# junipertcy/bipartiteSBM-MCMC

Measured on AMD Instinct MI355X. Metric: node-label MH updates/s, higher is better.
Workload: dtype f64

## Files before the change

bipartitesbm-mcmc_amd/build.py:

```python
import os
import shutil
import subprocess
import sys

HERE = os.path.dirname(os.path.abspath(__file__))
CSRC = os.path.join(HERE, "csrc")
LIB = os.path.join(HERE, "libbisbm_hip.so")
SOURCES = ["bisbm_kernels.hip", "bisbm_sweep_fast.hip", "bisbm_handle.hip", "bisbm_anneal.hip", "bisbm_marginals.hip",
           "bisbm_multi.hip", "bisbm_merge.hip", "bisbm_align.hip", "bisbm_tempering.hip", "bisbm_population.hip", "bisbm_pair_scores.hip", "bisbm_partition.hip",
           "bisbm_query_scores.hip", "bisbm_coassign.hip", "bisbm_foldin.hip", "bisbm_conditionals.hip", "bisbm_heatbath.hip", "bisbm_reshuffle.hip",
           "bisbm_mode_marginals.hip", "bisbm_trace.hip",
           "bisbm_tables.cpp", "bisbm_io.cpp"]
HEADERS = ["bisbm_device.hpp", "bisbm_partition_device.hpp", "bisbm_kernels.hpp", "bisbm_stand_rule.hpp", "bisbm_engine.hpp", "bisbm_pass_policy.hpp", os.path.join("..", "host", "bisbm.hpp"),
           os.path.join("..", "host", "mcmc_main.cpp"), os.path.join("..", "..", "include", "bisbm.h"),
           os.path.join("..", "..", "include", "bisbm_io.h")]
FLAGS = ["--offload-arch=gfx950", "-O3", "-std=c++17", "-ffp-contract=off", "-fPIC", "-pthread",
         "-Wall", "-Wno-unused-function",
         "-mllvm", "-structurizecfg-skip-uniform-regions=true",
         "-mllvm", "-amdgpu-atomic-optimizer-strategy=None",
         "-falign-loops=64"]


def hipcc():
    for cand in (shutil.which("hipcc"), "/opt/rocm/bin/hipcc"):
        if cand and os.path.exists(cand):
            return cand
    raise RuntimeError("hipcc not found: the engine is HIP-only and cannot be built without ROCm")


def needs_build():
    if not os.path.exists(LIB):
        return True
    t = os.path.getmtime(LIB)
    deps = [os.path.join(CSRC, s) for s in SOURCES + HEADERS] + [os.path.abspath(__file__)]
    return any(os.path.getmtime(d) > t for d in deps)


def build(force=False, verbose=False):
    import fcntl
    if not force and not needs_build():
        return LIB
    with open(os.path.join(HERE, ".build.lock"), "w") as lock:
        fcntl.flock(lock, fcntl.LOCK_EX)
        try:
            if not force and not needs_build():
                return LIB
# ... 100 lines not shown
```

bipartitesbm-mcmc_amd/csrc/bisbm_anneal.hip:

```cpp
#include "bisbm_engine.hpp"

using namespace bisbm;

extern "C" {

int bisbm_anneal(bisbm_handle h, int schedule, const float kwargs[2], uint64_t duration_steps,
                 uint64_t steps_await, double* acc_rate_out) {
    if (!h) return BISBM_ERR_INVALID_ARG;
    if (h->temper.L)
        return fail(h, BISBM_ERR_STATE, "replica exchange is on: sweeps run through bisbm_tempering_run (bisbm_tempering_set(h, 0, NULL) turns it off)");
    return anneal_engine(h, schedule, kwargs, duration_steps, steps_await, acc_rate_out, nullptr);
}

}

int bisbm::anneal_engine(bisbm_engine* h, int schedule, const float kwargs[2], uint64_t duration_steps, uint64_t steps_await,
                         double* acc_rate_out, const float* T_chain) {
    if (!kwargs) return fail(h, BISBM_ERR_INVALID_ARG, "kwargs is NULL");
    if (schedule < BISBM_SCHED_EXPONENTIAL || schedule > BISBM_SCHED_ABRUPT_COOL)
        return fail(h, BISBM_ERR_INVALID_ARG, "unknown schedule %d", schedule);
    if (!h->devs.empty()) return multi_anneal(h, schedule, kwargs, duration_steps, steps_await, acc_rate_out);
    if (!h->groups.empty()) {
        const size_t G = h->groups.size();
        std::vector<int> rcs(G, BISBM_OK);
// ... 181 lines not shown
            Slice sl;
            sl.T = schedule_table(sched, k0, k1, t0, len, &sl.zero_after);
            return sl;
        });
    };
    if (tab_segments) start_slice(0, slice_sweeps(sweeps_left));
    bool first = true;
    while (first || sweeps_left > 0) {
        if (segmented) {
            const uint64_t now = slice_sweeps(sweeps_left);
            p.duration = now * h->n;
            p.t_base = sweeps_done * h->n;
            p.resume = first ? 0u : 1u;
            if (tab_segments) {
                Slice sl;
                try {
                    sl = next_slice.get();
                } catch (...) {
                    return fail(h, BISBM_ERR_STATE, "temperature table: out of host memory");
                }
                if (int rc = upload_table(sl.T, p.t_base, sl.zero_after)) return rc;
            }
            sweeps_left -= now;
            sweeps_done += now;
        }
        first = false;
        uint32_t depth = max_depth;
        if (max_depth >= 2u) {
            depth = h->passes.choose(max_depth, h->n <= 100000);
            if (const char* pd = getenv("BISBM_PASS_DEPTH"))
                depth = pd[0] == '2' ? 1u : pd[0] == '4' ? std::min(2u, max_depth) : pd[0] == '8' ? max_depth : depth;
        }
        p.pass_depth = depth;
        {
            const uint32_t d = std::min(p.pair_steps, p.pass_depth);
            const bool cold = schedule == SCHED_CONSTANT && kwargs[0] == 0.f;
            h->last_pass_steps = (!fast || cold) ? 1u
                                 : (h->ka <= 8 && h->kb <= 8 && d >= 3u) ? 8u
                                 : (h->ka <= 32 && h->kb <= 32 && d >= 2u) ? 4u
                                 : p.pair_steps != 0u ? 2u : 1u;
        }
        HIPCHK(h, hipEventRecord(h->ev0, h->stream));
        if (fast)
            HIPCHK(h, launch_sweep_fast(p, lds, h->stream));
        else
            HIPCHK(h, launch_sweep(p, h->rng_mode, lds, h->stream));
        HIPCHK(h, hipEventRecord(h->ev1, h->stream));
        if (tab_segments && sweeps_left > 0) start_slice(sweeps_done, slice_sweeps(sweeps_left));
        HIPCHK(h, hipStreamSynchronize(h->stream));
        float ms = 0;
        HIPCHK(h, hipEventElapsedTime(&ms, h->ev0, h->ev1));
        ms_sum += ms;
        HIPCHK(h, hipMemcpy(sc.data(), h->d_scalars, sizeof(ChainScalars) * h->n_chains, hipMemcpyDeviceToHost));
        uint64_t upd = 0;
        bool all_stopped = true;
        for (uint32_t c = 0; c < h->n_chains; ++c) {
            acc_sum[c] += sc[c].last_accepted;
            sweeps_sum[c] += sc[c].last_sweeps;
            upd += sc[c].last_sweeps * h->n;
            all_stopped = all_stopped && sc[c].stopped != 0;
        }
        updates += upd;
        if (max_depth >= 2u && ms > 0.05f && upd > 0) {
            const double speed = (double)upd / ms;
            uint64_t acc_now = 0;
            for (uint32_t c = 0; c < h->n_chains; ++c) acc_now += sc[c].last_accepted;
            const double acc_frac = (double)acc_now / (double)upd;
            const double before[3] = {h->passes.figure(1), h->passes.figure(2), h->passes.figure(3)};
            const uint32_t incumbent = h->passes.current();
            h->passes.record(depth, speed, acc_frac);
            if (getenv("BISBM_PASS_LOG"))
                fprintf(stderr, "[bisbm passes] depth %u%s: %.3e updates/ms, accepted %.3f (before the launch: two %.3e, four %.3e, eight %.3e; incumbent %u -> %u)\n",
                        depth, depth != incumbent && incumbent != 0u && h->passes.settled() ? " (a look)" : "", speed, acc_frac, before[0], before[1], before[2],
                        incumbent, h->passes.current());
        }
        if (segmented && fast && all_stopped) {
            if (next_slice.valid()) next_slice.wait();
            break;
        }
    }
    const float ms = (float)ms_sum;
    h->last_kernel_ms = ms_sum;
    if (segmented) {
        for (uint32_t c = 0; c < h->n_chains; ++c) {
            sc[c].last_accepted = acc_sum[c];
            sc[c].last_sweeps = sweeps_sum[c];
            sc[c].last_rate = (fast && sc[c].stopped) ? (double)acc_sum[c] / (double)(sweeps_sum[c] * h->n)
                                                      : (double)acc_sum[c] / (double)duration_steps;
        }
        HIPCHK(h, hipMemcpy(h->d_scalars, sc.data(), sizeof(ChainScalars) * h->n_chains, hipMemcpyHostToDevice));
    }
    if (sum_from_entropy) {
        if (int rc = launch_block_entropy(h, h->d_tmp_f64)) return rc;
        HIPCHK(h, launch_sum_from_entropy(h->d_scalars, h->d_ent_prev, h->d_tmp_f64, h->n_chains, h->stream));
        HIPCHK(h, hipMemcpyAsync(h->d_ent_prev, h->d_tmp_f64, sizeof(double) * h->n_chains, hipMemcpyDeviceToDevice, h->stream));
        HIPCHK(h, hipStreamSynchronize(h->stream));
        h->ent_prev_valid = true;
    }
    for (uint32_t c = 0; c < h->n_chains; ++c)
        if (acc_rate_out) acc_rate_out[c] = sc[c].last_rate;
// ... 23 lines not shown
```

bipartitesbm-mcmc_amd/csrc/bisbm_engine.hpp:

```cpp
#pragma once

#include <hip/hip_runtime.h>

#include <algorithm>
#include <atomic>
#include <cmath>
#include <cstdarg>
#include <cstdio>
#include <cstdlib>
#include <cstring>
#include <future>
#include <limits>
#include <map>
#include <memory>
#include <mutex>
#include <queue>
#include <random>
#include <set>
#include <sstream>
#include <string>
#include <thread>
#include <utility>
#include <vector>

// ... 287 lines not shown
    uint8_t* d_labels_tmp = nullptr;
    size_t label_stride = 0;
    bool wide = false;
    size_t lbytes() const { return wide ? 2 : 1; }
    uint32_t* d_vlist = nullptr;
    int32_t* d_m = nullptr;
    int32_t* d_m_r = nullptr;
    int32_t* d_n_r = nullptr;
    uint32_t* d_eta = nullptr;
    bisbm::ChainScalars* d_scalars = nullptr;
    uint32_t* d_simd_claims = nullptr;
    uint32_t* d_mt_engine = nullptr;
    uint32_t* d_mt_gen = nullptr;
    double* d_lgamma = nullptr;
    double* d_logtab = nullptr;
    double* d_q = nullptr;
    bisbm::DeviceBuf<double> d_T;
    double* d_tmp_f64 = nullptr;
    double* d_ent_prev = nullptr;
    bool ent_prev_valid = false;
    uint32_t* d_stage_u32 = nullptr;
    uint32_t* d_counts = nullptr;
    uint32_t counts_kmax = 0;
    uint32_t counts_cols = 0;
    uint32_t cap_ka = 0, cap_kb = 0;
    std::shared_ptr<bisbm::HostTables> tab;
    uint32_t q_stride = 0;
    double ent_deg = 0, ent_multi = 0;
    std::shared_ptr<std::vector<uint64_t>> deg_count;
    double last_kernel_ms = 0;
    uint64_t last_updates = 0;
    uint32_t last_pass_steps = 0;
    bisbm::PassDepthPolicy passes;
    std::vector<bisbm_engine*> groups;
    std::vector<std::pair<uint32_t, uint32_t>> where;
    bisbm_engine* root = nullptr;
    std::vector<uint32_t> gids, ridx;
    uint32_t* d_gids = nullptr;
    uint32_t gid(size_t c) const { return gids.empty() ? first_chain_id + (uint32_t)c : gids[c]; }
    std::vector<bisbm_engine*> devs;
    std::vector<uint32_t> dev_first;
    struct DevicePool* pool = nullptr;
    uint64_t counts_rows = 0;
    bisbm::AlignState align;
    bisbm::TemperState temper;
    bisbm::PopulationState population;
    bisbm::PairScoreState pairs;
    bisbm::QueryScoreState queries;
    bisbm::CoassignState coassign;
    bisbm::FoldinState foldin;
    bisbm::ConditionalState cond;
    bisbm::ReshuffleState reshuffle;
    bisbm::PartitionState partition;
    bisbm::ModeState modes;
    bisbm::TraceState trace;
};

namespace bisbm {

extern thread_local std::string g_create_error;

int fail(bisbm_engine* h, int code, const char* fmt, ...) __attribute__((format(printf, 3, 4)));

#define HIPCHK(h, expr)                                                                              \
    do {                                                                                             \
        hipError_t e_ = (expr);                                                                      \
        if (e_ != hipSuccess) return fail((h), BISBM_ERR_HIP, "%s: %s", #expr, hipGetErrorString(e_)); \
    } while (0)

#define RESERVE(h, buf, count)                                                                                                \
    do {                                                                                                                      \
        const size_t n_ = (count);                                                                                            \
        hipError_t e_ = (buf).reserve(n_);                                                                                    \
        if (e_ != hipSuccess)                                                                                                 \
            return fail((h), BISBM_ERR_HIP, "%s: %zu bytes of device memory for " #buf " could not be allocated: %s", __func__, \
                        n_ * sizeof(*(buf).get()), hipGetErrorString(e_));                                                    \
    } while (0)

void free_chain_arrays(bisbm_engine* h);
void free_all(bisbm_engine* h);
void mt_seed_host(uint32_t* mt, uint64_t seed);
inline void philox_host(uint64_t seed, uint32_t chain, uint32_t purpose, uint64_t idx, uint32_t out[4]) {
    uint32_t c0 = (uint32_t)idx, c1 = (uint32_t)(idx >> 32), c2 = chain, c3 = purpose;
    uint32_t k0 = (uint32_t)seed, k1 = (uint32_t)(seed >> 32);
    for (int r = 0; r < 10; ++r) {
        const uint64_t p0 = (uint64_t)0xD2511F53u * c0, p1 = (uint64_t)0xCD9E8D57u * c2;
        const uint32_t n0 = (uint32_t)(p1 >> 32) ^ c1 ^ k0, n2 = (uint32_t)(p0 >> 32) ^ c3 ^ k1;
        c1 = (uint32_t)p1;
        c3 = (uint32_t)p0;
        c0 = n0;
        c2 = n2;
        k0 += 0x9E3779B9u;
        k1 += 0xBB67AE85u;
    }
    out[0] = c0, out[1] = c1, out[2] = c2, out[3] = c3;
}
inline double u53_host(uint32_t hi, uint32_t lo) { return (double)((((uint64_t)hi << 32) | lo) >> 11) * 0x1.0p-53; }
inline void forget_pass_speeds(bisbm_engine* h) { h->passes.reset(); }
int rebuild_state(bisbm_engine* h);
int launch_block_entropy(bisbm_engine* h, double* d_out);

template <class F>
int each_group(bisbm_engine* h, F f) {
    for (bisbm_engine* g : h->groups) {
        const int rc = f(g);
        if (rc) {
            h->err = g->err;
            return rc;
        }
    }
    return BISBM_OK;
}
bool common_shape(bisbm_engine* h);
int shared_shape(bisbm_engine* h, uint32_t* ka, uint32_t* kb);
template <class T, class F>
int gather_groups(bisbm_engine* h, T* out, F f) {
    return each_group(h, [&](bisbm_engine* g) {
        std::vector<T> tmp(g->n_chains);
        const int rc = f(g, tmp.data());
        if (rc == BISBM_OK && out)
            for (size_t j = 0; j < tmp.size(); ++j) out[g->ridx[j]] = tmp[j];
        return rc;
    });
}

size_t generic_lds_base_bytes(uint32_t ka, uint32_t kb, bool wide, int rng_mode);
constexpr size_t kLdsPerCu = 160 * 1024;

template <class F>
bool for_each_chain(size_t C, F&& fn) {
    std::atomic<bool> ok{true};
// ... 130 lines not shown
```

bipartitesbm-mcmc_amd/csrc/bisbm_kernels.hpp:

```cpp
#pragma once

#include <hip/hip_runtime.h>
#include <stdint.h>

#include "bisbm_device.hpp"

struct bisbm_reshuffle_record;

namespace bisbm {

struct ChainScalars {
    double cum_dS;
    double accu_r;
    double last_rate;
    uint64_t sweeps_total;
    uint64_t last_accepted;
    uint64_t last_sweeps;
    uint32_t shuffle_epoch;
    uint32_t engine_idx;
    uint32_t gen_idx;
    uint32_t merge_epoch;
    uint32_t hw_id[2];
    uint32_t xcc_id;
    uint32_t split_epoch;
// ... 13 lines not shown
    const uint32_t* chain_gids;
    uint8_t* labels;
    size_t label_stride;
    uint32_t* vlist;
    int32_t* m;
    int32_t* m_r;
    int32_t* n_r;
    uint32_t* eta;
    ChainScalars* scalars;
    uint32_t* mt_engine;
    uint32_t* mt_gen;
    const double* lgamma_tab;
    uint64_t lgamma_size;
    const double* q_tab;
    uint32_t q_stride;
    const double* log_tab;
    const double* T_tab;
    uint64_t T_len;
    uint64_t T_base;
    int T_zero_after;
    int schedule;
    float kw0, kw1;
    uint64_t duration, steps_await;
    uint64_t t_base, call_duration;
    uint32_t resume;
    uint64_t seed;
    int eta_in_lds;
    uint32_t eta_w, eta_lo_a, eta_lo_b;
    int vlist_in_lds;
    uint32_t* simd_claims;
    uint32_t fixed_stepping_wave;
    uint32_t pair_steps;
    uint32_t pass_depth;
    uint32_t wide;
    uint32_t keep_sum;
    const float* T_chain;
};
constexpr uint32_t kSimdClaims = 1u << 14;

struct BuildParams {
    const uint32_t* rowptr;
    const uint32_t* col;
    uint32_t n, na, ka, kb, maxdeg, n_chains;
    const uint8_t* labels;
    size_t label_stride;
    int32_t* m;
    int32_t* m_r;
    int32_t* n_r;
    uint32_t* eta;
    uint32_t wide;
};

struct ShuffleParams {
    uint32_t n, na, nb, n_chains, first_chain_id;
    const uint32_t* chain_gids;
    uint64_t seed;
    uint8_t* labels;
    const uint8_t* labels_old;
    size_t label_stride;
    ChainScalars* scalars;
    uint32_t* mt_engine;
    uint32_t wide;
};

struct EntropyParams {
    uint32_t ka, kb, maxdeg, n_chains;
    const int32_t* m;
    const int32_t* m_r;
    const int32_t* n_r;
    const uint32_t* eta;
// ... 373 lines not shown
```

bipartitesbm-mcmc_amd/csrc/bisbm_sweep_fast.hip:

```cpp
#include "bisbm_kernels.hpp"
#include "bisbm_stand_rule.hpp"

#include <algorithm>
#include <cstdio>
#include <type_traits>

namespace bisbm {

#ifdef BISBM_STAMPS
__device__ unsigned long long g_fast_stamps[16];
#define FSTAMP(i)                                                                        \
    do {                                                                                 \
        unsigned long long now_;                                                         \
        __builtin_amdgcn_sched_barrier(0);                                               \
        __asm__ volatile("s_memtime %0\n\ts_waitcnt lgkmcnt(0)" : "=s"(now_)::"memory"); \
        __builtin_amdgcn_sched_barrier(0);                                               \
        st_acc[i] += now_ - st_prev;                                                     \
        st_prev = now_;                                                                  \
    } while (0)
#else
#define FSTAMP(i) \
    do {          \
    } while (0)
#endif
#if defined(BISBM_STAMPS) && BISBM_STAMPS == 2
#define FSTAMP_STEP(i) \
    do {               \
    } while (0)
#else
#define FSTAMP_STEP(i) FSTAMP(i)
#endif

__device__ __forceinline__ void wfence() {
    __builtin_amdgcn_wave_barrier();
    __asm__ volatile("" ::: "memory");
}

__device__ __forceinline__ double tab_at(const double* base, uint32_t idx) {
#if defined(BISBM_ABLATE) && (BISBM_ABLATE & 8)
    return (double)idx * 1e-3 + (double)((size_t)base & 0xff);
#endif
    return *(const double*)((const char*)base + (uint32_t)(idx << 3));
}

struct __attribute__((packed, aligned(4))) Id4 {
    uint32_t x, y, z, w;
};

__device__ __forceinline__ uint32_t sflag(uint32_t x) {
    uint32_t r;
    __asm__("s_min_u32 %0, %1, 1" : "=s"(r) : "s"(x) : "scc");
    return r;
}
__device__ __forceinline__ uint32_t smin(uint32_t x, uint32_t y) {
    uint32_t r;
    __asm__("s_min_u32 %0, %1, %2" : "=s"(r) : "s"(x), "s"(y) : "scc");
    return r;
}


#ifdef BISBM_PASS_COUNTS
constexpr int kPassCounts = 13;
__device__ unsigned long long g_pass_counts[kPassCounts];
#define PCOUNT(i, v) (pc_acc[i] += (v))
#define PASS_COUNTS_PAIR(paired)                                                          \
    do {                                                                                  \
        const uint32_t pm_ = (paired) & chA, colk_ = col & sflag(kAtB) & (set_clash ^ 1u); \
        const uint32_t mv_ = target_moves(margin, kAtB);                                  \
        pc_acc[0] += 1u;                                                                  \
        pc_acc[1] += 1u + stands;                                                         \
        pc_acc[2] += pm_;                                                                 \
        pc_acc[3] += pm_ & set_clash;                                                     \
        pc_acc[4] += pm_ & colk_ & (mv_ ^ 1u);                                            \
        pc_acc[5] += pm_ & colk_ & mv_;                                                   \
        pc_acc[6] += pm_ & colk_ & (margin == kAtB ? 1u : 0u);                            \
        pc_acc[7] += pm_ & colk_ & (margin + 1u == kAtB ? 1u : 0u);                       \
    } while (0)
#else
#define PCOUNT(i, v) \
    do {             \
    } while (0)
#define PASS_COUNTS_PAIR(paired) \
    do {                         \
    } while (0)
#endif

#ifndef BISBM_PREDICT_TARGET
#define BISBM_PREDICT_TARGET 1
#endif
constexpr uint32_t kHistStride = 68;
constexpr uint32_t kHandWords = 9;
// ... 16 lines not shown
    double logn, tail_lg, L2_0, L2_1, L4_0, L4_1;
};

struct PairSteps {
    uint32_t r_locA, r_locB, degA, degB, t_locB, s_prdA, s_prdB;
    uint32_t liveA, liveB;
    uint32_t selfA, selfB, warmA, warmB;
    uint32_t prop, pack_v, deg, r_loc, t_loc;
    double u_acc;
    __device__ __forceinline__ uint32_t flags(uint32_t clash) const {
        return (liveA & (selfA ^ 1u)) | ((liveA & selfA & warmA) << 1) | ((liveB & (selfB ^ 1u)) << 2) | ((liveB & selfB & warmB) << 3) |
               (clash << 4);
    }
};

__device__ __forceinline__ uint32_t rows4(unsigned long long b) {
    const unsigned long long x = b >> 15;
    return (uint32_t)(x | (x >> 15) | (x >> 30) | (x >> 45)) & 0xfu;
}
__device__ __forceinline__ void commit_four(uint32_t nst, uint32_t clash_bits, uint32_t mv4, uint32_t& moved, uint32_t& commit) {
    const uint32_t c01 = (clash_bits >> 1) & 1u, c02 = (clash_bits >> 2) & 1u, c03 = (clash_bits >> 3) & 1u;
    const uint32_t c12 = (clash_bits >> 6) & 1u, c13 = (clash_bits >> 7) & 1u, c23 = (clash_bits >> 11) & 1u;
    const uint32_t m0 = mv4 & 1u;
    const uint32_t k1 = sflag(nst - 1u) & ((m0 & c01) ^ 1u);
    const uint32_t m1 = k1 & (mv4 >> 1) & 1u;
    const uint32_t k2 = k1 & (nst > 2u ? 1u : 0u) & ((m0 & c02) ^ 1u) & ((m1 & c12) ^ 1u);
    const uint32_t m2 = k2 & (mv4 >> 2) & 1u;
    const uint32_t k3 = k2 & (nst > 3u ? 1u : 0u) & ((m0 & c03) ^ 1u) & ((m1 & c13) ^ 1u) & ((m2 & c23) ^ 1u);
    const uint32_t m3 = k3 & (mv4 >> 3) & 1u;
    commit = 1u | (k1 << 1) | (k2 << 2) | (k3 << 3);
    moved = m0 | (m1 << 1) | (m2 << 2) | (m3 << 3);
}

template <bool EL, bool CT, bool K32, bool K16, bool K8, bool Q32>
__global__ __launch_bounds__(2 * kWave, 2) void sweep_fast_kernel(SweepParams p) {
    extern __shared__ __align__(16) uint32_t lds32[];
    const uint32_t chain = blockIdx.x;
    if (chain >= p.n_chains) return;
    const uint32_t lane = threadIdx.x & 63u;
    if (p.resume != 0u && p.scalars[chain].stopped != 0u) {
        if (threadIdx.x == 0) {
            p.scalars[chain].last_accepted = 0;
            p.scalars[chain].last_sweeps = 0;
        }
        return;
    }
    const uint32_t ka = p.ka, kb = p.kb, K = ka + kb, na = p.na, nb = p.nb;
    const uint32_t D = p.maxdeg + 1, S = kb | 1u;
    constexpr bool kPredictTarget = !K16 && !Q32 && (BISBM_PREDICT_TARGET != 0);
    const uint32_t row_cap = p.maxdeg < kRowCap ? p.maxdeg : kRowCap;
    const uint32_t o_mq = 0, o_eta = ka * S;
    const uint32_t eta_w = EL ? D : p.eta_w;
    const uint32_t o_hist8 = o_eta + (EL ? K * D : (ka > kb ? ka : kb) * eta_w);
    const uint32_t o_hand = o_hist8 + 2 * kWave * (kHistStride / 4);
    const uint32_t o_slow = o_hand + 2 * kHandWords * kWave;
    const uint32_t o_flag = o_slow + kWave;
    int32_t* const mq = (int32_t*)(lds32 + o_mq);
    uint32_t* const eta_l = lds32 + o_eta;
    uint32_t* const hist8_base = lds32 + o_hist8;
    uint32_t* const hand_base = lds32 + o_hand;
    int32_t* const slow_hist = (int32_t*)(lds32 + o_slow);
    uint32_t* const stop_flag = lds32 + o_flag;
    unsigned long long* const below1_total = (unsigned long long*)(lds32 + ((o_flag + 4u + 1u) & ~1u));
    const uint32_t wave_in_wg = (uint32_t)__builtin_amdgcn_readfirstlane((int)(threadIdx.x >> 6));
    uint32_t hw_id, xcc_id;
    __asm__ volatile("s_getreg_b32 %0, hwreg(HW_REG_HW_ID)" : "=s"(hw_id));
    __asm__ volatile("s_getreg_b32 %0, hwreg(HW_REG_XCC_ID)" : "=s"(xcc_id));
    uint32_t* const role = lds32 + o_flag + 1;
// ... 726 lines not shown
                    const uint32_t r_i = (uint32_t)__builtin_amdgcn_ds_bpermute(li, (int)r_c);
                    const uint32_t s_i = (uint32_t)__builtin_amdgcn_ds_bpermute(li, (int)s_c);
                    const uint32_t r_j = (uint32_t)__builtin_amdgcn_ds_bpermute(lj, (int)r_c);
                    const uint32_t s_j = (uint32_t)__builtin_amdgcn_ds_bpermute(lj, (int)s_c);
                    const uint32_t t_j = (uint32_t)__builtin_amdgcn_ds_bpermute(lj, (int)t_c);
                    const int at_sj = lj + (int)((s_j & 15u) << 2);
                    const uint32_t margins_j = (uint32_t)__builtin_amdgcn_ds_bpermute(at_sj, (int)m_c);
                    const uint32_t k_i_tj = k_of_i_at(li, t_j);
                    const uint32_t set_i = (1u << r_i) | (1u << s_i), set_j = (1u << r_j) | (1u << s_j);
                    const uint32_t in_between = column_clash<DEPTH>(r_i, s_i, s_j, k_i_tj, margins_j);
#ifdef BISBM_PASS_COUNTS
                    {
                        const uint32_t shared = (set_i & set_j) != 0u ? 1u : 0u;
                        const uint32_t cand = column_clash_any(r_i, s_i, s_j, k_i_tj) & (shared ^ 1u);
                        const uint32_t margin = packed_margin(margins_j, r_i < s_i ? 1u : 0u), need = (DEPTH - 1u) * k_i_tj;
                        pc_pair_code = shared | (cand << 1) | ((cand & in_between) << 2) | ((cand & (need == margin ? 1u : 0u)) << 3) |
                                       ((cand & (need == margin + 1u ? 1u : 0u)) << 4);
                    }
#endif
                    return __builtin_amdgcn_ballot_w64(((set_i & set_j) | in_between) != 0u);
                };
#ifdef BISBM_PASS_COUNTS
                auto count_pairs = [&](uint32_t i, uint32_t j, bool pair_lane, uint32_t moved, uint32_t commit, uint32_t nst) {
                    const bool on = pair_lane && i < j && j < nst && ((moved >> i) & 1u) != 0u && ((commit >> ((j - 1u) & 7u)) & 1u) != 0u;
                    const uint32_t c = on ? pc_pair_code : 0u;
                    pc_acc[8] += (unsigned)__builtin_popcountll(__builtin_amdgcn_ballot_w64((c & 1u) != 0u));
                    pc_acc[9] += (unsigned)__builtin_popcountll(__builtin_amdgcn_ballot_w64((c & 6u) == 2u));
                    pc_acc[10] += (unsigned)__builtin_popcountll(__builtin_amdgcn_ballot_w64((c & 6u) == 6u));
                    pc_acc[11] += (unsigned)__builtin_popcountll(__builtin_amdgcn_ballot_w64((c & 8u) != 0u));
                    pc_acc[12] += (unsigned)__builtin_popcountll(__builtin_amdgcn_ballot_w64((c & 16u) != 0u));
                };
#endif
                auto apply_moves = [&](auto tm, auto width, uint32_t q, uint32_t qs, uint32_t grp_l, uint32_t moved, uint32_t selfok, uint32_t r_loc,
                                       uint32_t s_loc, uint32_t deg, double dS, uint32_t e_idx, int ee, auto&& write_mq) {
                    constexpr bool TM = decltype(tm)::value;
                    constexpr uint32_t W = decltype(width)::value, L = 64u / W;
                    constexpr unsigned long long kFirst = W == 4u ? 0x0001000100010001ull : 0x0101010101010101ull;
                    acc_chunk += (uint32_t)__builtin_popcount(moved | selfok);
                    if ((TM ? (moved | selfok) : moved) != 0u) {
                        const unsigned long long movers = __builtin_amdgcn_ballot_w64(((moved >> grp_l) & 1u) != 0u);
                        wfence();
                        write_mq(movers);
                        if (__builtin_amdgcn_inverse_ballot_w64(movers & (kFirst * 0x30ull)))
                            eta_l[e_idx] = (uint32_t)(ee + ((int)(lb & 1u) * 2 - 1));
                        if (__builtin_amdgcn_inverse_ballot_w64(movers & kFirst)) new_lab[qs] = (uint8_t)(own_base + s_loc);
#pragma unroll
                        for (uint32_t g = 0; g < W; ++g) {
                            if ((moved >> g) & 1u) {
                                const uint32_t rg = readlane(r_loc, L * g), sg = readlane(s_loc, L * g), dg = readlane(deg, L * g);
                                const int dl = (int)min(lb ^ rg, 1u) - (int)min(lb ^ sg, 1u);
                                mr_own += __mul24((int)dg, dl);
                                nr_own += dl;
                                if constexpr (TM) cum_l0 += readlane(dS, L * g + L - 1u);
                                if constexpr (TM) new_minimum(q + g);
                            } else if (TM && ((selfok >> g) & 1u)) {
                                new_minimum(q + g);
                            }
                        }
                        wfence();
                    }
                };
                auto multi_loop = [&](auto tm, auto width, auto&& pass) {
                    constexpr uint32_t W = decltype(width)::value;
                    uint32_t q = 0;
                    acc_chunk = 0;
                    while (q < cnt) {
                        const uint32_t some = (uint32_t)(gen_mask >> q) & ((1u << W) - 1u);
                        if (__builtin_expect((some & 1u) != 0u, 0)) {
                            step_general(q, T_of_step(q));
                            q += 1u;
                        } else {
                            const uint32_t nst = min(min((uint32_t)__builtin_ctz(some | (1u << W)), W), cnt - q);
                            const uint32_t done = pass(tm, q, nst);
                            PCOUNT(0, 1u);
                            PCOUNT(1, done);
                            q += done;
                        }
                    }
                    acc_l0 += (unsigned long long)acc_chunk;
                };

                auto step_pair = [&](auto tm, uint32_t q, uint32_t pairable) -> uint32_t {
                    const uint32_t qB = q + pairable;
                    const uint32_t qs = q + ((uint32_t)half_mask_l & pairable);
                    FSTAMP_STEP(0);
                    PairSteps P = pair_head(q, qB, qs, pairable);
                    const uint32_t r_locA = P.r_locA, s_prdA = P.s_prdA, r_locB = P.r_locB, s_prdB = P.s_prdB, t_locB = P.t_locB;
                    const uint32_t prop = P.prop, deg = P.deg, r_loc = P.r_loc, t_loc = P.t_loc;
                    const int k = (int)hist8_cur[qs * kHistStride + lb];
// ... 222 lines not shown
                    const unsigned long long m_warm = CT ? ~0ull : ~__builtin_amdgcn_ballot_w64(((zeroT_mask >> qs) & 1ull) != 0ull);
                    const unsigned long long b_can = m_valid & m_live & ~m_self & kRowRep;
                    const unsigned long long b_selfok = m_valid & m_live & m_self & m_warm & kRowRep;
                    if (b_can == 0ull) {
                        acc_chunk += (uint32_t)__builtin_popcountll(b_selfok);
                        if constexpr (TM)
                            if (b_selfok != 0ull) new_minimum(q + ((uint32_t)__builtin_ctzll(b_selfok) >> 4));
                        return nst;
                    }
                    TargetReads t;
                    target_lds(t, s_loc, r_loc, deg, kmask);
                    target_gathers(t, kk, std::false_type{});
                    const double a0 = k * (t.m_st + eps) * inv_blk;
                    const double a1 = k * (m_rt - k + eps) * inv_blk;
                    const double accu0 = butterfly_rows16(a0);
                    const double accu1 = butterfly_rows16(a1);
                    const double lq = hot_log_q(std::true_type{}, t.qn, t.qk, t.logn);
                    const uint32_t clash_bits =
                        (uint32_t)clash_pairs(Four{}, r_loc, s_loc, t_loc, pack_margins(margin_up((uint32_t)scan, (uint32_t)w_piv, prop), margin_down((uint32_t)scan, prop)),
                                              (int)(((lane >> 2) & 3u) << 6), (int)((lane & 3u) << 6), [&](int li, uint32_t t_j) {
                            return (uint32_t)__builtin_amdgcn_ds_bpermute(li + (int)(t_j << 2), (int)kk);
                        }) & 0xffffu;
                    double d = (L1 + t.L2) - (L3 + t.L4);
                    d = d + t.tail_lg * sign_tail;
                    d = d + lq * sign_q;
                    const double dS = butterfly_rows16(d);
                    const unsigned long long b_acc = accept_rows(dS, accu0, accu1, u_acc, qs, m_warm, b_can);
                    const uint32_t mv4 = rows4(b_can & b_acc), selfok4 = rows4(b_selfok);
                    uint32_t moved, commit;
                    commit_four(nst, clash_bits, mv4, moved, commit);
#ifdef BISBM_PASS_COUNTS
                    count_pairs((lane >> 2) & 3u, lane & 3u, lane < 16u, moved, commit, nst);
#endif
                    apply_moves(tm, Four{}, q, qs, row, moved, commit & selfok4, r_loc, s_loc, deg, dS, t.e_idx, t.ee, [&](unsigned long long movers) {
                        if (__builtin_amdgcn_inverse_ballot_w64(movers & lanes_koth)) {
                            mq[a_rt] = m_rt_raw - k;
                            mq[t.a_st] = t.m_st_raw + k;
                        }
                    });
                    return (uint32_t)__builtin_popcount(commit);
                };
                auto step_quad32 = [&](auto tm, uint32_t q, uint32_t nst) -> uint32_t {
                    constexpr bool TM = decltype(tm)::value;
                    const uint32_t qs = q + min(row, nst - 1u);
                    const int sel = (int)(qs << 2);
                    const uint32_t prop = prop_of(qs);
                    const uint32_t pack = (uint32_t)__builtin_amdgcn_ds_bpermute(sel, (int)pack_l);
                    const double u_acc = u_acc_of(qs);
                    const uint32_t deg = pack & 255u, r_loc = (pack >> 8) & 63u, t_loc = (pack >> 16) & 63u;
                    const int k0 = (int)hist8_cur[qs * kHistStride + l16], k1 = (int)hist8_cur[qs * kHistStride + l16 + 16u];
                    const uint32_t a_rt0 = mq_at(r_loc, l16), a_rt1 = mq_at(r_loc, l16 + 16u);
                    const int32_t m_rt_raw0 = mq[a_rt0], m_rt_raw1 = mq[a_rt1];
                    const int w0 = mq[mq_at(l16, t_loc)], w1 = mq[mq_at(l16 + 16u, t_loc)];
                    const int nn_r = __builtin_amdgcn_ds_bpermute((int)(r_loc << 2), nr_own);
                    const int32_t kmask0 = (0 - k0) >> 31, kmask1 = (0 - k1) >> 31;
                    const int32_t m_rt0 = m_rt_raw0 & kmask0, m_rt1 = m_rt_raw1 & kmask1;
                    const uint32_t kk0 = (uint32_t)k0, kk1 = (uint32_t)k1;
                    const double L1_0 = tab_at(tab.lg, (uint32_t)(m_rt0 + 1)), L3_0 = tab_at(tab.lg, (uint32_t)(m_rt0 + 1) - kk0);
                    const double L1_1 = tab_at(tab.lg, (uint32_t)(m_rt1 + 1)), L3_1 = tab_at(tab.lg, (uint32_t)(m_rt1 + 1) - kk1);
                    __asm__ volatile("" ::: "memory");
                    const int scan0 = row_inclusive_scan16(w0);
                    int tot = w0;
                    tot += __builtin_amdgcn_update_dpp(0, tot, kDppXor1, 0xF, 0xF, false);
                    tot += __builtin_amdgcn_update_dpp(0, tot, kDppXor2, 0xF, 0xF, false);
                    tot += __builtin_amdgcn_update_dpp(0, tot, kDppHalfMirror, 0xF, 0xF, false);
                    tot += __builtin_amdgcn_update_dpp(0, tot, kDppMirror, 0xF, 0xF, false);
                    const int scan1 = row_inclusive_scan16(w1) + tot;
// ... 4 lines not shown
                    const unsigned long long m_valid = nst >= 4u ? ~0ull : ((1ull << (16u * nst)) - 1ull);
                    const unsigned long long m_live = __builtin_amdgcn_ballot_w64(nn_r != 1);
                    const unsigned long long m_self = __builtin_amdgcn_ballot_w64(s_loc == r_loc);
                    const unsigned long long m_warm = CT ? ~0ull : ~__builtin_amdgcn_ballot_w64(((zeroT_mask >> qs) & 1ull) != 0ull);
                    const unsigned long long b_can = m_valid & m_live & ~m_self & kRowRep;
                    const unsigned long long b_selfok = m_valid & m_live & m_self & m_warm & kRowRep;
                    if (b_can == 0ull) {
                        acc_chunk += (uint32_t)__builtin_popcountll(b_selfok);
                        if constexpr (TM)
                            if (b_selfok != 0ull) new_minimum(q + ((uint32_t)__builtin_ctzll(b_selfok) >> 4));
                        return nst;
                    }
                    TargetReads2 t;
                    target_lds2(t, s_loc, r_loc, deg, kmask0, kmask1, l16, 16u);
                    target_gathers2(t, kk0, kk1, std::true_type{});
                    const uint32_t leaf_m = 0u - (s_loc >> 4);
                    const uint32_t S_own = (uint32_t)scan0 ^ (((uint32_t)scan0 ^ (uint32_t)scan1) & leaf_m);
                    const uint32_t w_own = (uint32_t)w0 ^ (((uint32_t)w0 ^ (uint32_t)w1) & leaf_m);
                    uint32_t margins = pack_margins(margin_up(S_own, w_own, prop), margin_down(S_own, prop));
                    __asm__ volatile("" : "+v"(margins));
                    const double a0 = k0 * (t.m_st0 + eps) * invq_lo + k1 * (t.m_st1 + eps) * invq_hi;
                    const double a1 = k0 * (m_rt0 - k0 + eps) * invq_lo + k1 * (m_rt1 - k1 + eps) * invq_hi;
                    const double accu0 = butterfly_rows16(a0);
                    const double accu1 = butterfly_rows16(a1);
                    const double lq = hot_log_q(std::false_type{}, t.qn, t.qk, t.logn);
                    const uint32_t clash_bits =
                        (uint32_t)clash_pairs(Four{}, r_loc, s_loc, t_loc, margins,
                                              (int)(((lane >> 2) & 3u) << 6), (int)((lane & 3u) << 6), [&](int li, uint32_t t_j) {
                            const int src = li + (int)((t_j & 15u) << 2);
                            const uint32_t k_lo = (uint32_t)__builtin_amdgcn_ds_bpermute(src, (int)kk0);
                            const uint32_t k_hi = (uint32_t)__builtin_amdgcn_ds_bpermute(src, (int)kk1);
                            return k_lo ^ ((k_lo ^ k_hi) & (0u - (t_j >> 4)));
                        }) & 0xffffu;
                    double d0 = (L1_0 + t.L2_0) - (L3_0 + t.L4_0);
                    d0 = d0 + t.tail_lg * sign_tail;
                    d0 = d0 + lq * sign_q;
                    const double d1 = (L1_1 + t.L2_1) - (L3_1 + t.L4_1);
                    const double dS = butterfly_rows16(d1) + butterfly_rows16(d0);
                    const unsigned long long b_acc = accept_rows(dS, accu0, accu1, u_acc, qs, m_warm, b_can);
                    const uint32_t mv4 = rows4(b_can & b_acc), selfok4 = rows4(b_selfok);
                    uint32_t moved, commit;
                    commit_four(nst, clash_bits, mv4, moved, commit);
#ifdef BISBM_PASS_COUNTS
                    count_pairs((lane >> 2) & 3u, lane & 3u, lane < 16u, moved, commit, nst);
#endif
                    apply_moves(tm, Four{}, q, qs, row, moved, commit & selfok4, r_loc, s_loc, deg, dS, t.e_idx, t.ee, [&](unsigned long long movers) {
                        if (__builtin_amdgcn_inverse_ballot_w64(movers & lanes_koth32_lo)) {
                            mq[a_rt0] = m_rt_raw0 - k0;
                            mq[t.a_st0] = t.m_st_raw0 + k0;
                        }
                        if (__builtin_amdgcn_inverse_ballot_w64(movers & lanes_koth32_hi)) {
                            mq[a_rt1] = m_rt_raw1 - k1;
                            mq[t.a_st1] = t.m_st_raw1 + k1;
                        }
                    });
                    return (uint32_t)__builtin_popcount(commit);
                };
                const uint32_t grp = lane >> 3;
                auto step_oct = [&](auto tm, uint32_t q, uint32_t nst) -> uint32_t {
                    constexpr bool TM = decltype(tm)::value;
                    const uint32_t qs = q + min(grp, nst - 1u);
                    const int sel = (int)(qs << 2);
                    const uint32_t prop = prop_of(qs);
                    const uint32_t pack = (uint32_t)__builtin_amdgcn_ds_bpermute(sel, (int)pack_l);
                    const double u_acc = u_acc_of(qs);
                    const uint32_t deg = pack & 255u, r_loc = (pack >> 8) & 63u, t_loc = (pack >> 16) & 63u;
                    const int k = (int)hist8_cur[qs * kHistStride + lb];
                    const uint32_t a_rt = mq_at(r_loc, lb);
                    const int32_t m_rt_raw = mq[a_rt];
                    const int w_piv = mq[mq_at(lb, t_loc)];
                    const int nn_r = __builtin_amdgcn_ds_bpermute((int)(r_loc << 2), nr_own);
                    const int32_t kmask = (0 - k) >> 31;
                    const int32_t m_rt = m_rt_raw & kmask;
                    const uint32_t kk = (uint32_t)k;
                    const double L1 = tab_at(tab.lg, (uint32_t)(m_rt + 1));
                    const double L3 = tab_at(tab.lg, (uint32_t)(m_rt + 1) - kk);
                    __asm__ volatile("" ::: "memory");
                    const int scan = group_inclusive_scan8(w_piv, lb);
                    const unsigned long long hit = __builtin_amdgcn_ballot_w64((uint32_t)scan > prop);
// ... 13 lines not shown
                        return nst;
                    }
                    TargetReads t;
                    target_lds(t, s_loc, r_loc, deg, kmask);
                    target_gathers(t, kk, std::false_type{});
                    const double a0 = k * (t.m_st + eps) * inv_blk;
                    const double a1 = k * (m_rt - k + eps) * inv_blk;
                    const double accu0 = butterfly_groups8(a0);
                    const double accu1 = butterfly_groups8(a1);
                    const double lq = hot_log_q(std::true_type{}, t.qn, t.qk, t.logn);
                    const unsigned long long clash_bits =
                        clash_pairs(Eight{}, r_loc, s_loc, t_loc, pack_margins(margin_up((uint32_t)scan, (uint32_t)w_piv, prop), margin_down((uint32_t)scan, prop)),
                                    (int)((lane & 7u) << 5), (int)((lane >> 3) << 5), [&](int li, uint32_t t_j) {
                            return (uint32_t)__builtin_amdgcn_ds_bpermute(li + (int)(t_j << 2), (int)kk);
                        });
                    double d = (L1 + t.L2) - (L3 + t.L4);
                    d = d + t.tail_lg * sign_tail;
                    d = d + lq * sign_q;
                    const double dS = butterfly_groups8(d);
                    const unsigned long long b_acc = accept_rows(dS, accu0, accu1, u_acc, qs, m_warm, b_can);
                    auto groups8 = [](unsigned long long b) -> uint32_t { return (uint32_t)(((b >> 7) * 0x0102040810204080ull) >> 56) & 0xffu; };
                    const uint32_t mv8 = groups8(b_can & b_acc), selfok8 = groups8(b_selfok);
                    uint32_t moved = mv8 & 1u, commit = 1u, stands = 1u;
#pragma unroll
                    for (uint32_t j = 1; j < 8u; ++j) {
                        const uint32_t clash_j = (uint32_t)(clash_bits >> (8u * j)) & moved;
                        stands &= (nst > j ? 1u : 0u) & (clash_j == 0u ? 1u : 0u);
                        commit |= stands << j;
                        moved |= (stands & (mv8 >> j) & 1u) << j;
                    }
#ifdef BISBM_PASS_COUNTS
                    count_pairs(lane & 7u, lane >> 3, true, moved, commit, nst);
#endif
                    apply_moves(tm, Eight{}, q, qs, grp, moved, commit & selfok8, r_loc, s_loc, deg, dS, t.e_idx, t.ee, [&](unsigned long long movers) {
                        if (__builtin_amdgcn_inverse_ballot_w64(movers & lanes_koth)) {
                            mq[a_rt] = m_rt_raw - k;
                            mq[t.a_st] = t.m_st_raw + k;
                        }
                    });
                    return (uint32_t)__builtin_popcount(commit);
                };
                auto pair_loop = [&](auto tm) {
                    uint32_t q = 0;
                    acc_chunk = 0;
                    while (q < cnt) {
                        const uint32_t two = (uint32_t)(gen_mask >> q) & 3u;
                        if (__builtin_expect((two & 1u) != 0u, 0)) {
                            step_general(q, T_of_step(q));
                            q += 1u;
                        } else if (K32) {
                            q += step_pair(tm, q, ((two >> 1) ^ 1u) & sflag(cnt - 1u - q));
                        } else {
                            const uint32_t done = step_pair64(tm, q, ((two >> 1) ^ 1u) & sflag(cnt - 1u - q) & (pair64_mode ? 1u : 0u));
                            if constexpr (kPredictTarget) {
                                if (__builtin_expect(done == 0u, 0)) gen_mask |= 1ull << q;
                            }
                            q += done;
                        }
                    }
                    acc_l0 += (unsigned long long)acc_chunk;
                };
                if constexpr (!K32) {
                    if (track_min != 0u)
                        pair_loop(std::true_type{});
                    else
                        pair_loop(std::false_type{});
                } else if (K8 && oct_mode) {
// ... 80 lines not shown
    for (uint32_t i = lane; i < ka * kb; i += kWave) m_g[i] = mq[(i / kb) * S + (i % kb)];
    if (lane < ka) {
        mr_g[lane] = mrA;
        nr_g[lane] = nrA;
    }
    if (lane < kb) {
        mr_g[ka + lane] = mrB;
        nr_g[ka + lane] = nrB;
    }
    if (EL)
        for (uint32_t i = lane; i < K * D; i += kWave) eta_g[i] = eta_l[i];
#ifdef BISBM_STAMPS
    if (lane == 0)
        for (int i = 0; i < 12; ++i) atomicAdd(&g_fast_stamps[i], st_acc[i]);
#endif
#ifdef BISBM_PASS_COUNTS
    if (lane == 0)
        for (int i = 0; i < kPassCounts; ++i) atomicAdd(&g_pass_counts[i], pc_acc[i]);
#endif
    if (lane == 0) {
        if (track_min != 0u) sc->cum_dS = cum_l0;
        sc->sweeps_total = sweeps_total;
        sc->last_rate = rate;
        sc->last_accepted = acc_l0;
        sc->last_sweeps = sweeps_done;
        sc->stop_emin = emin_l0;
        sc->stop_mark = mark_l0;
        sc->stop_below1 = *below1_total;
        sc->stopped = stopped ? 1u : 0u;
        if (p.simd_claims != nullptr) atomicSub(&p.simd_claims[role[wave_in_wg]], 1u);
    }
}

template <bool EL, bool CT, bool K32, bool K16, bool K8, bool Q32 = false>
static hipError_t launch_fast_variant3(const SweepParams& p, size_t lds_bytes, hipStream_t stream) {
    hipError_t e = hipFuncSetAttribute((const void*)sweep_fast_kernel<EL, CT, K32, K16, K8, Q32>,
                                       hipFuncAttributeMaxDynamicSharedMemorySize, (int)lds_bytes);
    if (e != hipSuccess) return e;
    hipLaunchKernelGGL((sweep_fast_kernel<EL, CT, K32, K16, K8, Q32>), dim3(p.n_chains), dim3(2 * kWave), lds_bytes, stream, p);
    return hipGetLastError();
}

template <bool EL, bool CT>
hipError_t launch_fast_variant(const SweepParams& p, size_t lds_bytes, hipStream_t stream) {
    const uint32_t depth = p.pair_steps < p.pass_depth ? p.pair_steps : p.pass_depth;
    if (p.ka <= 8u && p.kb <= 8u && depth >= 3u) return launch_fast_variant3<EL, CT, true, true, true>(p, lds_bytes, stream);
    if (p.ka <= 16u && p.kb <= 16u && depth >= 2u) return launch_fast_variant3<EL, CT, true, true, false>(p, lds_bytes, stream);
    if (p.ka <= 32u && p.kb <= 32u && depth >= 2u) return launch_fast_variant3<EL, CT, true, false, false, true>(p, lds_bytes, stream);
    return (p.ka <= 32u && p.kb <= 32u) ? launch_fast_variant3<EL, CT, true, false, false>(p, lds_bytes, stream)
                                        : launch_fast_variant3<EL, CT, false, false, false>(p, lds_bytes, stream);
}

#ifndef BISBM_FAST_PART
#define BISBM_FAST_PART -1
#endif
#define BISBM_FAST_HERE(part) (BISBM_FAST_PART == -1 || BISBM_FAST_PART == (part))
#if BISBM_FAST_HERE(0)
template hipError_t launch_fast_variant<false, false>(const SweepParams&, size_t, hipStream_t);
#endif
#if BISBM_FAST_HERE(1)
template hipError_t launch_fast_variant<false, true>(const SweepParams&, size_t, hipStream_t);
#endif
#if BISBM_FAST_HERE(2)
template hipError_t launch_fast_variant<true, false>(const SweepParams&, size_t, hipStream_t);
#endif
#if BISBM_FAST_HERE(3)
template hipError_t launch_fast_variant<true, true>(const SweepParams&, size_t, hipStream_t);
#endif

#if BISBM_FAST_HERE(4)
#if BISBM_FAST_PART == 4
extern template hipError_t launch_fast_variant<false, false>(const SweepParams&, size_t, hipStream_t);
extern template hipError_t launch_fast_variant<false, true>(const SweepParams&, size_t, hipStream_t);
extern template hipError_t launch_fast_variant<true, false>(const SweepParams&, size_t, hipStream_t);
extern template hipError_t launch_fast_variant<true, true>(const SweepParams&, size_t, hipStream_t);
#endif

size_t sweep_fast_lds_bytes(uint32_t ka, uint32_t kb, uint32_t maxdeg, bool eta_in_lds, uint32_t eta_window) {
    const uint32_t K = ka + kb, D = maxdeg + 1, S = kb | 1u;
    const size_t dwords = (size_t)ka * S + (eta_in_lds ? (size_t)K * D : (size_t)std::max(ka, kb) * eta_window) +
                          2 * (size_t)kWave * (kHistStride / 4) + 2 * (size_t)kHandWords * kWave + kWave + 4 + 10 + 16 + 64 + 128;
// ... 48 lines not shown
```

Before: 2.189 billion.

## Add one-stage quad32 kernel combining move deltas via permlane swaps at high acceptance

```diff
diff --git a/bipartitesbm-mcmc_amd/build.py b/bipartitesbm-mcmc_amd/build.py
--- a/bipartitesbm-mcmc_amd/build.py
+++ b/bipartitesbm-mcmc_amd/build.py
@@ -11,7 +11,7 @@
            "bisbm_query_scores.hip", "bisbm_coassign.hip", "bisbm_foldin.hip", "bisbm_conditionals.hip", "bisbm_heatbath.hip", "bisbm_reshuffle.hip",
            "bisbm_mode_marginals.hip", "bisbm_trace.hip",
            "bisbm_tables.cpp", "bisbm_io.cpp"]
-HEADERS = ["bisbm_device.hpp", "bisbm_partition_device.hpp", "bisbm_kernels.hpp", "bisbm_stand_rule.hpp", "bisbm_engine.hpp", "bisbm_pass_policy.hpp", os.path.join("..", "host", "bisbm.hpp"),
+HEADERS = ["bisbm_device.hpp", "bisbm_partition_device.hpp", "bisbm_kernels.hpp", "bisbm_stand_rule.hpp", "bisbm_move_word.hpp", "bisbm_engine.hpp", "bisbm_pass_policy.hpp", os.path.join("..", "host", "bisbm.hpp"),
            os.path.join("..", "host", "mcmc_main.cpp"), os.path.join("..", "..", "include", "bisbm.h"),
            os.path.join("..", "..", "include", "bisbm_io.h")]
 FLAGS = ["--offload-arch=gfx950", "-O3", "-std=c++17", "-ffp-contract=off", "-fPIC", "-pthread",
diff --git a/bipartitesbm-mcmc_amd/csrc/bisbm_anneal.hip b/bipartitesbm-mcmc_amd/csrc/bisbm_anneal.hip
--- a/bipartitesbm-mcmc_amd/csrc/bisbm_anneal.hip
+++ b/bipartitesbm-mcmc_amd/csrc/bisbm_anneal.hip
@@ -237,6 +237,8 @@
                 depth = pd[0] == '2' ? 1u : pd[0] == '4' ? std::min(2u, max_depth) : pd[0] == '8' ? max_depth : depth;
         }
         p.pass_depth = depth;
+        p.one_stage = h->last_acc_frac >= kOneStageAccepted ? 1u : 0u;
+        if (const char* os = getenv("BISBM_ONE_STAGE")) p.one_stage = os[0] == '1' ? 1u : 0u;
         {
             const uint32_t d = std::min(p.pair_steps, p.pass_depth);
             const bool cold = schedule == SCHED_CONSTANT && kwargs[0] == 0.f;
@@ -271,6 +273,7 @@
             uint64_t acc_now = 0;
             for (uint32_t c = 0; c < h->n_chains; ++c) acc_now += sc[c].last_accepted;
             const double acc_frac = (double)acc_now / (double)upd;
+            h->last_acc_frac = acc_frac;
             const double before[3] = {h->passes.figure(1), h->passes.figure(2), h->passes.figure(3)};
             const uint32_t incumbent = h->passes.current();
             h->passes.record(depth, speed, acc_frac);
diff --git a/bipartitesbm-mcmc_amd/csrc/bisbm_engine.hpp b/bipartitesbm-mcmc_amd/csrc/bisbm_engine.hpp
--- a/bipartitesbm-mcmc_amd/csrc/bisbm_engine.hpp
+++ b/bipartitesbm-mcmc_amd/csrc/bisbm_engine.hpp
@@ -343,6 +343,7 @@
     uint64_t last_updates = 0;
     uint32_t last_pass_steps = 0;
     bisbm::PassDepthPolicy passes;
+    double last_acc_frac = -1.;
     std::vector<bisbm_engine*> groups;
     std::vector<std::pair<uint32_t, uint32_t>> where;
     bisbm_engine* root = nullptr;
@@ -407,7 +408,10 @@
     out[0] = c0, out[1] = c1, out[2] = c2, out[3] = c3;
 }
 inline double u53_host(uint32_t hi, uint32_t lo) { return (double)((((uint64_t)hi << 32) | lo) >> 11) * 0x1.0p-53; }
-inline void forget_pass_speeds(bisbm_engine* h) { h->passes.reset(); }
+inline void forget_pass_speeds(bisbm_engine* h) {
+    h->passes.reset();
+    h->last_acc_frac = -1.;
+}
 int rebuild_state(bisbm_engine* h);
 int launch_block_entropy(bisbm_engine* h, double* d_out);
 
diff --git a/bipartitesbm-mcmc_amd/csrc/bisbm_kernels.hpp b/bipartitesbm-mcmc_amd/csrc/bisbm_kernels.hpp
--- a/bipartitesbm-mcmc_amd/csrc/bisbm_kernels.hpp
+++ b/bipartitesbm-mcmc_amd/csrc/bisbm_kernels.hpp
@@ -69,10 +69,12 @@
     uint32_t fixed_stepping_wave;
     uint32_t pair_steps;
     uint32_t pass_depth;
+    uint32_t one_stage;
     uint32_t wide;
     uint32_t keep_sum;
     const float* T_chain;
 };
+constexpr double kOneStageAccepted = 0.7;
 constexpr uint32_t kSimdClaims = 1u << 14;
 
 struct BuildParams {
diff --git a/bipartitesbm-mcmc_amd/csrc/bisbm_move_word.hpp b/bipartitesbm-mcmc_amd/csrc/bisbm_move_word.hpp
--- /dev/null
+++ b/bipartitesbm-mcmc_amd/csrc/bisbm_move_word.hpp
@@ -0,0 +1,25 @@
+#pragma once
+
+#include <cstdint>
+
+#include "bisbm_stand_rule.hpp"
+
+namespace bisbm {
+
+BISBM_RULE_FN int32_t move_word(uint32_t r, uint32_t s, uint32_t deg, uint32_t b) {
+    const int32_t at_s = (int32_t)((deg << 2) | 1u), at_r = (int32_t)((0u - (deg << 2)) | 3u);
+    return b == s ? at_s : (b == r ? at_r : 0);
+}
+BISBM_RULE_FN int32_t move_word_dn(int32_t z) { return (int32_t)((uint32_t)z << 30) >> 30; }
+BISBM_RULE_FN int32_t move_word_dm(int32_t z) { return z >> 2; }
+
+template <class V, class Ops>
+BISBM_RULE_FN V combine_move_words(V z_lo, V z_hi, const Ops& ops) {
+    V x, y;
+    ops.swap16(z_lo, z_hi, x, y);
+    const V rows = x | y;
+    ops.swap32(rows, rows, x, y);
+    return x | y;
+}
+
+}
diff --git a/bipartitesbm-mcmc_amd/csrc/bisbm_sweep_fast.hip b/bipartitesbm-mcmc_amd/csrc/bisbm_sweep_fast.hip
--- a/bipartitesbm-mcmc_amd/csrc/bisbm_sweep_fast.hip
+++ b/bipartitesbm-mcmc_amd/csrc/bisbm_sweep_fast.hip
@@ -1,4 +1,5 @@
 #include "bisbm_kernels.hpp"
+#include "bisbm_move_word.hpp"
 #include "bisbm_stand_rule.hpp"
 
 #include <algorithm>
@@ -57,6 +58,17 @@
     __asm__("s_min_u32 %0, %1, %2" : "=s"(r) : "s"(x), "s"(y) : "scc");
     return r;
 }
+
+struct LaneSwaps {
+    __device__ __forceinline__ void swap16(int a, int b, int& x, int& y) const {
+        const auto r = __builtin_amdgcn_permlane16_swap(a, b, false, false);
+        x = (int)r[0], y = (int)r[1];
+    }
+    __device__ __forceinline__ void swap32(int a, int b, int& x, int& y) const {
+        const auto r = __builtin_amdgcn_permlane32_swap(a, b, false, false);
+        x = (int)r[0], y = (int)r[1];
+    }
+};
 
 
 #ifdef BISBM_PASS_COUNTS
@@ -139,8 +151,8 @@
     moved = m0 | (m1 << 1) | (m2 << 2) | (m3 << 3);
 }
 
-template <bool EL, bool CT, bool K32, bool K16, bool K8, bool Q32>
-__global__ __launch_bounds__(2 * kWave, 2) void sweep_fast_kernel(SweepParams p) {
+template <bool EL, bool CT, bool K32, bool K16, bool K8, bool Q32, bool OS>
+__device__ __forceinline__ void sweep_fast_body(const SweepParams& p) {
     extern __shared__ __align__(16) uint32_t lds32[];
     const uint32_t chain = blockIdx.x;
     if (chain >= p.n_chains) return;
@@ -933,7 +945,8 @@
                 };
 #endif
                 auto apply_moves = [&](auto tm, auto width, uint32_t q, uint32_t qs, uint32_t grp_l, uint32_t moved, uint32_t selfok, uint32_t r_loc,
-                                       uint32_t s_loc, uint32_t deg, double dS, uint32_t e_idx, int ee, auto&& write_mq) {
+                                       uint32_t s_loc, uint32_t deg, auto combined, int zw_lo, int zw_hi, double dS, uint32_t e_idx, int ee,
+                                       auto&& write_mq) {
                     constexpr bool TM = decltype(tm)::value;
                     constexpr uint32_t W = decltype(width)::value, L = 64u / W;
                     constexpr unsigned long long kFirst = W == 4u ? 0x0001000100010001ull : 0x0101010101010101ull;
@@ -945,17 +958,28 @@
                         if (__builtin_amdgcn_inverse_ballot_w64(movers & (kFirst * 0x30ull)))
                             eta_l[e_idx] = (uint32_t)(ee + ((int)(lb & 1u) * 2 - 1));
                         if (__builtin_amdgcn_inverse_ballot_w64(movers & kFirst)) new_lab[qs] = (uint8_t)(own_base + s_loc);
+                        if constexpr (decltype(combined)::value) {
+                            static_assert(W == 4u, "rows of 16 lanes");
+                            const bool mover_lane = __builtin_amdgcn_inverse_ballot_w64(movers);
+                            const int z = combine_move_words(mover_lane ? zw_lo : 0, mover_lane ? zw_hi : 0, LaneSwaps{});
+                            mr_own += move_word_dm(z);
+                            nr_own += move_word_dn(z);
+                        }
+                        if constexpr (TM || !decltype(combined)::value) {
 #pragma unroll
-                        for (uint32_t g = 0; g < W; ++g) {
-                            if ((moved >> g) & 1u) {
-                                const uint32_t rg = readlane(r_loc, L * g), sg = readlane(s_loc, L * g), dg = readlane(deg, L * g);
-                                const int dl = (int)min(lb ^ rg, 1u) - (int)min(lb ^ sg, 1u);
-                                mr_own += __mul24((int)dg, dl);
-                                nr_own += dl;
-                                if constexpr (TM) cum_l0 += readlane(dS, L * g + L - 1u);
-                                if constexpr (TM) new_minimum(q + g);
-                            } else if (TM && ((selfok >> g) & 1u)) {
-                                new_minimum(q + g);
+                            for (uint32_t g = 0; g < W; ++g) {
+                                if ((moved >> g) & 1u) {
+                                    if constexpr (!decltype(combined)::value) {
+                                        const uint32_t rg = readlane(r_loc, L * g), sg = readlane(s_loc, L * g), dg = readlane(deg, L * g);
+                                        const int dl = (int)min(lb ^ rg, 1u) - (int)min(lb ^ sg, 1u);
+                                        mr_own += __mul24((int)dg, dl);
+                                        nr_own += dl;
+                                    }
+                                    if constexpr (TM) cum_l0 += readlane(dS, L * g + L - 1u);
+                                    if constexpr (TM) new_minimum(q + g);
+                                } else if (TM && ((selfok >> g) & 1u)) {
+                                    new_minimum(q + g);
+                                }
                             }
                         }
                         wfence();
@@ -1244,7 +1268,7 @@
 #ifdef BISBM_PASS_COUNTS
                     count_pairs((lane >> 2) & 3u, lane & 3u, lane < 16u, moved, commit, nst);
 #endif
-                    apply_moves(tm, Four{}, q, qs, row, moved, commit & selfok4, r_loc, s_loc, deg, dS, t.e_idx, t.ee, [&](unsigned long long movers) {
+                    apply_moves(tm, Four{}, q, qs, row, moved, commit & selfok4, r_loc, s_loc, deg, std::false_type{}, 0, 0, dS, t.e_idx, t.ee, [&](unsigned long long movers) {
                         if (__builtin_amdgcn_inverse_ballot_w64(movers & lanes_koth)) {
                             mq[a_rt] = m_rt_raw - k;
                             mq[t.a_st] = t.m_st_raw + k;
@@ -1315,6 +1339,11 @@
                             const uint32_t k_hi = (uint32_t)__builtin_amdgcn_ds_bpermute(src, (int)kk1);
                             return k_lo ^ ((k_lo ^ k_hi) & (0u - (t_j >> 4)));
                         }) & 0xffffu;
+                    int zw_lo = 0, zw_hi = 0;
+                    if constexpr (OS) {
+                        zw_lo = move_word(r_loc, s_loc, deg, l16), zw_hi = move_word(r_loc, s_loc, deg, l16 + 16u);
+                        __asm__ volatile("" : "+v"(zw_lo), "+v"(zw_hi));
+                    }
                     double d0 = (L1_0 + t.L2_0) - (L3_0 + t.L4_0);
                     d0 = d0 + t.tail_lg * sign_tail;
                     d0 = d0 + lq * sign_q;
@@ -1327,7 +1356,7 @@
 #ifdef BISBM_PASS_COUNTS
                     count_pairs((lane >> 2) & 3u, lane & 3u, lane < 16u, moved, commit, nst);
 #endif
-                    apply_moves(tm, Four{}, q, qs, row, moved, commit & selfok4, r_loc, s_loc, deg, dS, t.e_idx, t.ee, [&](unsigned long long movers) {
+                    apply_moves(tm, Four{}, q, qs, row, moved, commit & selfok4, r_loc, s_loc, deg, std::bool_constant<OS>{}, zw_lo, zw_hi, dS, t.e_idx, t.ee, [&](unsigned long long movers) {
                         if (__builtin_amdgcn_inverse_ballot_w64(movers & lanes_koth32_lo)) {
                             mq[a_rt0] = m_rt_raw0 - k0;
                             mq[t.a_st0] = t.m_st_raw0 + k0;
@@ -1407,7 +1436,7 @@
 #ifdef BISBM_PASS_COUNTS
                     count_pairs(lane & 7u, lane >> 3, true, moved, commit, nst);
 #endif
-                    apply_moves(tm, Eight{}, q, qs, grp, moved, commit & selfok8, r_loc, s_loc, deg, dS, t.e_idx, t.ee, [&](unsigned long long movers) {
+                    apply_moves(tm, Eight{}, q, qs, grp, moved, commit & selfok8, r_loc, s_loc, deg, std::false_type{}, 0, 0, dS, t.e_idx, t.ee, [&](unsigned long long movers) {
                         if (__builtin_amdgcn_inverse_ballot_w64(movers & lanes_koth)) {
                             mq[a_rt] = m_rt_raw - k;
                             mq[t.a_st] = t.m_st_raw + k;
@@ -1554,13 +1583,25 @@
     }
 }
 
+template <bool EL, bool CT, bool K32, bool K16, bool K8, bool Q32>
+__global__ __launch_bounds__(2 * kWave, 2) void sweep_fast_kernel(SweepParams p) {
+    sweep_fast_body<EL, CT, K32, K16, K8, Q32, false>(p);
+}
+template <bool EL, bool CT>
+__global__ __launch_bounds__(2 * kWave, 2) void sweep_quad32_one_stage_kernel(SweepParams p) {
+    sweep_fast_body<EL, CT, true, false, false, true, true>(p);
+}
+
+template <class Kernel>
+static hipError_t launch_fast_kernel(Kernel kernel, const SweepParams& p, size_t lds_bytes, hipStream_t stream) {
+    hipError_t e = hipFuncSetAttribute((const void*)kernel, hipFuncAttributeMaxDynamicSharedMemorySize, (int)lds_bytes);
+    if (e != hipSuccess) return e;
+    hipLaunchKernelGGL(kernel, dim3(p.n_chains), dim3(2 * kWave), lds_bytes, stream, p);
+    return hipGetLastError();
+}
 template <bool EL, bool CT, bool K32, bool K16, bool K8, bool Q32 = false>
 static hipError_t launch_fast_variant3(const SweepParams& p, size_t lds_bytes, hipStream_t stream) {
-    hipError_t e = hipFuncSetAttribute((const void*)sweep_fast_kernel<EL, CT, K32, K16, K8, Q32>,
-                                       hipFuncAttributeMaxDynamicSharedMemorySize, (int)lds_bytes);
-    if (e != hipSuccess) return e;
-    hipLaunchKernelGGL((sweep_fast_kernel<EL, CT, K32, K16, K8, Q32>), dim3(p.n_chains), dim3(2 * kWave), lds_bytes, stream, p);
-    return hipGetLastError();
+    return launch_fast_kernel(sweep_fast_kernel<EL, CT, K32, K16, K8, Q32>, p, lds_bytes, stream);
 }
 
 template <bool EL, bool CT>
@@ -1568,7 +1609,9 @@
     const uint32_t depth = p.pair_steps < p.pass_depth ? p.pair_steps : p.pass_depth;
     if (p.ka <= 8u && p.kb <= 8u && depth >= 3u) return launch_fast_variant3<EL, CT, true, true, true>(p, lds_bytes, stream);
     if (p.ka <= 16u && p.kb <= 16u && depth >= 2u) return launch_fast_variant3<EL, CT, true, true, false>(p, lds_bytes, stream);
-    if (p.ka <= 32u && p.kb <= 32u && depth >= 2u) return launch_fast_variant3<EL, CT, true, false, false, true>(p, lds_bytes, stream);
+    if (p.ka <= 32u && p.kb <= 32u && depth >= 2u)
+        return p.one_stage != 0u ? launch_fast_kernel(sweep_quad32_one_stage_kernel<EL, CT>, p, lds_bytes, stream)
+                                 : launch_fast_variant3<EL, CT, true, false, false, true>(p, lds_bytes, stream);
     return (p.ka <= 32u && p.kb <= 32u) ? launch_fast_variant3<EL, CT, true, false, false>(p, lds_bytes, stream)
                                         : launch_fast_variant3<EL, CT, false, false, false>(p, lds_bytes, stream);
 }
```

Result: faster. 2.303 billion (median of 6 runs) (+5.2%).
